# dranov/raft-tla

Measured on AMD Instinct MI355X. Metric: distinct states/sec (node) on Raft BFS, higher is better.
Workload: dtype u32

## Files before the change

raft-tla_amd/csrc/orig_backend.hip:

```cpp
#include <hip/hip_runtime.h>

#include <algorithm>
#include <chrono>
#include <cstdio>
#include <cstdlib>
#include <cstring>
#include <functional>
#include <map>
#include <sstream>
#include <type_traits>

#include "../../include/raftmc.h"
#include "backend.h"
#include "chunk_plan.h"
#include "fp_gap.h"
#include "orig_spec.h"
#include "orig_text.h"
#include "rccl_api.h"
#include "shard_transport.h"
#include "sim_rng.h"
#include "state_store.h"

namespace rmc {

enum {
  K_NEW = 0, K_GEN_IN = 1, K_ERR = 2, K_EVENT = 3, K_ERRGID = 4, K_INS = 5, K_CHUNK_NEW = 6, K_LEVEL_NEW = 7,
  K_ACT = 8, K_PROF = K_ACT + 2 * OA_NACT,
  K_PROBES = K_PROF + 6,
  K_LEAD = K_PROF + 7,
  K_NCTR = K_PROF + 8
};
enum { EV_NEXT_ERROR = 0, EV_DEADLOCK = 1, EV_INV_ERROR = 2, EV_VIOLATION = 3 };
enum { OE_CAP_STORE = 0x100, OE_TABLE_FULL = 0x200 };
constexpr int DEDUP_PER = 4;
constexpr int BS = 256;
constexpr int LDS_FP_SLOTS = 2048;
constexpr int MAT_CAP = 2048;
#ifndef RMC_RV_PATCH
#define RMC_RV_PATCH 0
#endif
#ifndef RMC_RV_WCOUNT
#define RMC_RV_WCOUNT 0
#endif
constexpr int SCAN_BS = 1024;

template <int B, int E, class F>
__device__ __forceinline__ void static_for(F&& f) {
  if constexpr (B < E) {
    f(std::integral_constant<int, B>{});
    static_for<B + 1, E>(f);
  }
}

RMC_HD u64 ev_word(u64 gid, u32 inst, u32 kind) { return (((gid << 8) | (u64)inst) << 2) | (u64)kind; }

struct GenArgs {
  const u32* states;
  u64 chunk_begin, chunk_count;
  u64 gid0;
  u64* rfp;
  unsigned short* rkey;
  u32* rcnt;
  u64 seed;
  OrigRuntime rt;
  u32 inv_oom, deadlock;
  unsigned long long* ctr;
  u32* lead;
};

template <class S>
__global__ void __launch_bounds__(BS) __attribute__((amdgpu_waves_per_eu(S::NW <= 15 ? 4 : 1))) orig_generate(GenArgs a) {
  using W = typename S::Work;
  constexpr int NW = S::NW, NWP = (S::NW + 3) & ~3;
  __shared__ unsigned int lds_cnt[OA_NACT + 1];
  for (int t = threadIdx.x; t < OA_NACT + 1; t += BS) lds_cnt[t] = 0;
  __syncthreads();
  const u64 tid = (u64)blockIdx.x * BS + threadIdx.x;
  const bool active = tid < a.chunk_count;
  const u64 gid = a.gid0 + tid;
  const int lane = __lane_id();
  const u32 wave = __builtin_amdgcn_readfirstlane(threadIdx.x >> 6);
  const u64 wreg = (u64)blockIdx.x * (BS * S::NI) + (u64)wave * (64 * S::NI);
  u64* rfp = a.rfp + wreg;
  unsigned short* rkey = a.rkey + wreg;
  u32 wcount = 0;
  W s;
  u64 al[S::AW];
  u32 err = 0, nsucc = 0, nin = 0;
  unsigned long long ev = ~0ull;
  constexpr bool INC = NW <= 16;
  u32 bw[INC ? NW : 1];
  FpBase<INC ? NW : 2> fb;
  if (active) {
    u32 w[NWP];
    const uint4* src = reinterpret_cast<const uint4*>(a.states + (a.chunk_begin + tid) * NWP);
#pragma unroll
    for (int q = 0; q < NWP / 4; ++q) { const uint4 v = src[q]; w[4 * q] = v.x; w[4 * q + 1] = v.y; w[4 * q + 2] = v.z; w[4 * q + 3] = v.w; }
    S::unpack(w, s);
    S::all_logs_next(s, al);
  } else {
    S::init(s);
#pragma unroll
    for (int q = 0; q < S::AW; ++q) al[q] = 0;
// ... 527 lines not shown
    }
  }
  u64 wm[WW];
  u32 mine = 0;
#pragma unroll
  for (int q = 0; q < WW; ++q) { wm[q] = win[threadIdx.x * WW + q]; mine += (u32)__popcll(wm[q]); }
  u32 total = 0;
  const u32 off = block_excl_scan(mine, wave_tot, &total);
  if (threadIdx.x == 0) base_sh = total ? atomicAdd(&a.ctr[K_CHUNK_NEW], (unsigned long long)total) : 0ull;
  __syncthreads();
  u64 o = base_sh + off;
  const u64 pg = a.gid0 + (u64)blockIdx.x * BS + threadIdx.x;
#pragma unroll
  for (int q = 0; q < WW; ++q) {
    u64 m = wm[q];
    while (m) {
      const int k = q * 64 + __ffsll((unsigned long long)m) - 1;
      m &= m - 1;
      a.newpos[o++] = (pg << 8) | (u64)k;
    }
  }
  if (err) atomicOr(&a.ctr[K_ERR], (unsigned long long)err);
}

struct MatPlainArgs {
  u32* states;
  u64* meta;
  const u64* newrec;
  u64 base;
  u64 dst_base, cap;
  OrigRuntime rt;
  unsigned long long* ctr;
  u32 store;
};

template <class S>
__global__ void __launch_bounds__(BS) orig_materialize_plain(MatPlainArgs a) {
  using W = typename S::Work;
  constexpr int NW = S::NW, NWP = (S::NW + 3) & ~3;
  __shared__ unsigned int lds_cnt[OA_NACT];
  for (int t = threadIdx.x; t < OA_NACT; t += BS) lds_cnt[t] = 0;
  __syncthreads();
  const u64 n_new = a.ctr[K_CHUNK_NEW];
  const u64 base = a.dst_base + a.ctr[K_LEVEL_NEW];
  u32 err = 0;
  unsigned long long ev = ~0ull;
  for (u64 i = (u64)blockIdx.x * BS + threadIdx.x; i < n_new; i += (u64)gridDim.x * BS) {
    const u64 rec = a.newrec[i], pgid = rec >> 8;
    const int k = (int)(rec & 0xff);
    u32 w[NWP];
    const uint4* src = reinterpret_cast<const uint4*>(a.states + (pgid - a.base) * NWP);
#pragma unroll
    for (int q = 0; q < NWP / 4; ++q) { const uint4 v = src[q]; w[4 * q] = v.x; w[4 * q + 1] = v.y; w[4 * q + 2] = v.z; w[4 * q + 3] = v.w; }
    W s, t;
    u64 al[S::AW];
    S::unpack(w, s);
    S::all_logs_next(s, al);
    u32 e2 = 0;
    const int act = S::apply(s, k, t, e2);
#pragma unroll
    for (int q = 0; q < S::AW; ++q) t.allLogs[q] = al[q];
    u32 pw[NW];
    S::pack(t, pw);
    const u64 dst = base + i;
    if (act >= 0 && (!a.store || dst < a.cap)) {
      if (a.store) {
        uint4* o = reinterpret_cast<uint4*>(a.states + dst * NWP);
#pragma unroll
        for (int q = 0; q < NWP / 4; ++q)
          o[q] = make_uint4(pw[4 * q], 4 * q + 1 < NW ? pw[4 * q + 1] : 0u, 4 * q + 2 < NW ? pw[4 * q + 2] : 0u, 4 * q + 3 < NW ? pw[4 * q + 3] : 0u);
        a.meta[dst] = (pgid << 24) | ((u64)act << 16) | (u64)k;
      }
      atomicAdd(&lds_cnt[act], 1u);
      if (S::violated(t, a.rt.invariants & S::inv_frame(act))) { const u64 e = ev_word(pgid, (u32)k, EV_VIOLATION); ev = e < ev ? e : ev; }
    } else {
      err |= dst >= a.cap ? (u32)OE_CAP_STORE : (u32)OE_TABLE_FULL;
    }
  }
  if (err) atomicOr(&a.ctr[K_ERR], (unsigned long long)err);
  if (ev != ~0ull) atomicMin(&a.ctr[K_EVENT], ev);
  __syncthreads();
  for (int t = threadIdx.x; t < OA_NACT; t += BS)
    if (lds_cnt[t]) atomicAdd(&a.ctr[K_ACT + OA_NACT + t], (unsigned long long)lds_cnt[t]);
}

struct MarkArgs {
  const u64* newpos;
  const u64* table;
  u64 gid0, chunk_count;
  u64* winmask;
  u32 ww;
  unsigned long long* ctr;
};

__global__ void __launch_bounds__(BS) orig_mark(MarkArgs a) {
  const u64 n = a.ctr[K_INS];
  for (u64 i = (u64)blockIdx.x * BS + threadIdx.x; i < n; i += (u64)gridDim.x * BS) {
    const u64 key = ~a.table[2 * a.newpos[i] + 1];
    const u64 p = (key >> 8) - a.gid0;
    const u32 k = (u32)(key & 255);
    if (p >= a.chunk_count) { atomicOr(&a.ctr[K_ERR], (unsigned long long)OE_TABLE_FULL); continue; }
    atomicOr((unsigned long long*)&a.winmask[p * a.ww + (k >> 6)], 1ull << (k & 63));
  }
}

template <int WW>
__global__ void __launch_bounds__(BS) orig_count(const u64* winmask, u64 chunk_count, u32* wcnt) {
  __shared__ u32 wave_tot[BS / 64];
  const u64 p = (u64)blockIdx.x * BS + threadIdx.x;
  u32 mine = 0;
#pragma unroll
  for (int q = 0; q < WW; ++q) mine += p < chunk_count ? (u32)__popcll(winmask[p * WW + q]) : 0u;
  u32 total = 0;
  (void)block_excl_scan(mine, wave_tot, &total);
  if (threadIdx.x == 0) wcnt[blockIdx.x] = total;
}

__global__ void __launch_bounds__(SCAN_BS) orig_scan(const u32* wcnt, u64* woff, u32 nblk, unsigned long long* ctr) {
  __shared__ unsigned long long part[SCAN_BS];
  const u32 per = (nblk + SCAN_BS - 1) / SCAN_BS, b0 = threadIdx.x * per;
  unsigned long long s = 0;
  for (u32 j = 0; j < per; ++j) if (b0 + j < nblk) s += wcnt[b0 + j];
  part[threadIdx.x] = s;
  __syncthreads();
  for (int d = 1; d < SCAN_BS; d <<= 1) {
    const unsigned long long x = threadIdx.x >= (unsigned)d ? part[threadIdx.x - d] : 0ull;
    __syncthreads();
    part[threadIdx.x] += x;
    __syncthreads();
  }
  unsigned long long run = part[threadIdx.x] - s;
  for (u32 j = 0; j < per; ++j) if (b0 + j < nblk) { woff[b0 + j] = run; run += wcnt[b0 + j]; }
  if (threadIdx.x == SCAN_BS - 1) ctr[K_CHUNK_NEW] = part[SCAN_BS - 1];
}

struct MatArgs {
  u32* states;
  u64* meta;
  u64 chunk_begin, chunk_count, gid0;
  u64* winmask;
  const u64* woff;
  u32 ww;
  u64 dst_base, cap;
  OrigRuntime rt;
  unsigned long long* ctr;
};

template <class S>
__global__ void __launch_bounds__(BS) orig_materialize(MatArgs a) {
  using W = typename S::Work;
  constexpr int NW = S::NW, NWP = (S::NW + 3) & ~3, WW = (S::NI + 63) / 64;
  __shared__ unsigned int lds_cnt[OA_NACT];
  __shared__ unsigned short items[MAT_CAP];
  __shared__ u32 wave_tot[BS / 64];
  for (int t = threadIdx.x; t < OA_NACT; t += BS) lds_cnt[t] = 0;
  const u64 p = (u64)blockIdx.x * BS + threadIdx.x;
  u64 wm[WW];
  u32 mine = 0;
#pragma unroll
  for (int q = 0; q < WW; ++q) {
    wm[q] = p < a.chunk_count ? a.winmask[p * WW + q] : 0ull;
    mine += (u32)__popcll(wm[q]);
  }
  if (p < a.chunk_count && mine) {
#pragma unroll
    for (int q = 0; q < WW; ++q) a.winmask[p * WW + q] = 0ull;
// ... 673 lines not shown
    if (u32 bad = S::violated(s0, m_.rt.invariants)) {
      r.verdict = MC_VERDICT_INVARIANT_VIOLATION; r.violated = first_violated(bad);
      r.trace.push_back({"<Initial predicate>", state_text(s0, true)});
      r.seconds_total = std::chrono::duration<double>(std::chrono::steady_clock::now() - t0).count();
      return 0;
    }
    struct Dev { unsigned long long* ctr = nullptr; hipEvent_t e0 = nullptr, e1 = nullptr; DevOwner<HipDevApi> own; } d;
    HIPCHK(d.own.device(&d.ctr, SK_NCTR * 8));
    HIPCHK(d.own.event(&d.e0));
    HIPCHK(d.own.event(&d.e1));
    u64 h[SK_NCTR], event = ~0ull, maxlen = 1;
    for (u64 w0 = 0; w0 < num && event == ~0ull; w0 += batch) {
      const u64 n = std::min<u64>(batch, num - w0);
      std::memset(h, 0, sizeof h);
      h[SK_EVENT] = ~0ull;
      HIPCHK(hipMemcpy(d.ctr, h, sizeof h, hipMemcpyHostToDevice));
      SimArgs a;
      a.walk0 = w0; a.nwalks = n; a.seed = o.seed; a.depth = depth; a.rt = m_.rt;
      a.inv_oom = o.inv_out_of_model ? 1u : 0u; a.deadlock = o.check_deadlock ? 1u : 0u; a.ctr = d.ctr;
      HIPCHK(hipEventRecord(d.e0, nullptr));
      hipLaunchKernelGGL((orig_simulate<S>), dim3((unsigned)((n + BS - 1) / BS)), dim3(BS), 0, nullptr, a);
      HIPCHK(hipGetLastError());
      HIPCHK(hipEventRecord(d.e1, nullptr));
      HIPCHK(hipMemcpy(h, d.ctr, sizeof h, hipMemcpyDeviceToHost));
      float ms = 0;
      HIPCHK(hipEventElapsedTime(&ms, d.e0, d.e1));
      r.kernels[0].ms += ms; r.kernels[0].launches += 1; r.n_launches += 1;
      r.seconds_kernels += ms * 1e-3;
      r.sim_walks_run += (int64_t)n;
      r.sim_steps += (int64_t)h[SK_STEPS];
      for (int k = 0; k < OA_NACT; ++k) { r.act_generated[k] += (int64_t)h[SK_ACT + k]; r.generated += (int64_t)h[SK_ACT + k]; }
      maxlen = std::max<u64>(maxlen, h[SK_MAXLEN]);
      if (progress_)
        std::fprintf(stderr, "simulation: walks %llu..%llu, %llu steps, %.3f ms\n", (unsigned long long)w0,
                     (unsigned long long)(w0 + n - 1), (unsigned long long)h[SK_STEPS], ms);
      if (h[SK_ERR]) {
        r.verdict = MC_VERDICT_CAPACITY_OVERFLOW;
        r.error = (h[SK_ERR] & OE_CAP_ELECTIONS) ? "elections set exceeds the compiled capacity" : "message count outside the packed range";
        r.depth = (int64_t)maxlen;
        r.seconds_total = std::chrono::duration<double>(std::chrono::steady_clock::now() - t0).count();
        return 0;
      }
      event = h[SK_EVENT];
    }
    r.depth = (int64_t)maxlen;
    if (event != ~0ull) {
      const u64 walk = sim_event_walk(event);
      SimWalk<S> w;
      sim_replay<S>(m_.rt, o.inv_out_of_model, o.check_deadlock, o.seed, walk, depth, w);
      if (w.event != event) {
        err = "simulation: the host replay of walk " + std::to_string(walk) + " does not reproduce the device's event";
        return MC_E_STATE;
      }
      r.sim_event_walk = (int64_t)walk;
      const u32 kind = sim_event_kind(event);
      if (kind == EV_VIOLATION) {
        r.verdict = MC_VERDICT_INVARIANT_VIOLATION;
        r.violated = first_violated(S::violated(w.states.back(), m_.rt.invariants));
      } else if (kind == EV_DEADLOCK) {
        r.verdict = MC_VERDICT_DEADLOCK;
      } else {
        r.verdict = MC_VERDICT_EVAL_ERROR;
        r.error = "TLC evaluation error while computing the successors of the last state of walk " + std::to_string(walk) +
                  ": log[i][prevLogIndex] applied outside its domain (raft_original.tla:207-210)";
      }
      for (size_t k = 0; k < w.states.size(); ++k)
        r.trace.push_back({k == 0 ? std::string("<Initial predicate>") : std::string(kOrigActNames[w.acts[k - 1]]), state_text(w.states[k], true)});
    } else {
      r.verdict = MC_VERDICT_OK;
    }
    r.seconds_total = std::chrono::duration<double>(std::chrono::steady_clock::now() - t0).count();
    return 0;
  }

  struct Search {
    std::chrono::steady_clock::time_point t0;
    bool fifo = false;
    bool count_probes = false;
    bool count_last = false;
    u64* tbl = nullptr;
    u64 tmask = 0, full_mask = 0, st_slots = 0;
    u64 level_begin = 0, level_count = 1;
    ChunkPlan plan{0, 0, 0};
    bool last = false, ovl = false;
    int nch = 0;
    u64 nnew = 0;
    double level_ms = 0;
    u64 level_end() const { return level_begin + level_count; }
  };

  int run(const RunOpts& o, RunResult& r, std::string& err) override {
    if (o.sim_walks > 0) return simulate(o, r, err);
    unstored_ = 0;
    if (int rc = ensure_alloc(o, 0, err)) return rc;
    Search s;
    s.t0 = std::chrono::steady_clock::now();
    s.fifo = o.workers == 1;
    last_fifo_ = s.fifo;
    s.count_probes = std::getenv("RAFTMC_COUNT_PROBES") != nullptr;
    if (int rc = begin_search(o, s, err)) return rc;
    r = new_result(bfs_seed(o), {"orig_generate", "orig_merge_probe", "orig_mark_scan", "orig_materialize"});
    store_.reset();
    bool ended = false;
    if (int rc = init_level0(o, s, r, ended, err)) return rc;
    if (ended) return 0;
    s.count_last = o.count_final_level && !s.fifo && o.max_depth > 0 && o.checkpoint_path.empty();
    unstored_ = 0;
    const u64 sub_env = env_u64("RAFTMC_OVERLAP_STATES", ~0ull);
    s.plan = ChunkPlan(chunk_states_, s.fifo ? 0 : sub_env == ~0ull ? ChunkPlan::default_sub(chunk_states_) : sub_env,
                       env_u64("RAFTMC_OVERLAP_MIN_LEVEL", sub_env == ~0ull ? OVERLAP_MIN_LEVEL : 0), BS);
    const u64 S_B = NWP * 4;
    while (s.level_count > 0) {
      if (o.max_depth && r.depth >= o.max_depth) { r.left_on_queue = (int64_t)s.level_count; r.verdict = MC_VERDICT_DEPTH_LIMIT; break; }
      s.last = s.count_last && r.depth + 1 >= o.max_depth;
      if (int rc = maybe_spill(s, r, err)) return rc;
      if (!ctr_clean_) {
        hipLaunchKernelGGL(orig_reset_ctr, dim3(1), dim3(64), 0, stream_, (unsigned long long*)d_ctr_);
        HIPCHK(hipGetLastError());
      }
      ctr_clean_ = false;
      if (int rc = maybe_switch_to_full_table(s, r, err)) return rc;
      if (int rc = queue_level(o, s, r, err)) return rc;
      if (int rc = read_level(s, r, err)) return rc;
      u64* const c = h_ctr_;
      const u64 level_end = s.level_end(), nnew = s.nnew;
      if (!s.last && level_end + nnew - store_.base() > store_.cap()) c[K_ERR] |= OE_CAP_STORE;
      const bool event = c[K_EVENT] != ~0ull && (c[K_ERR] & ~(u64)OE_CAP_STORE) == 0;
      if (event && !s.fifo) return research_fifo(o, c[K_EVENT], r, err);
      if (event) {
        const u64 stored = std::min<u64>(nnew, store_.cap() - std::min<u64>(store_.cap(), level_end - store_.base()));
        bool decided = false;
        if (int rc = handle_event(c[K_EVENT], s.level_begin, s.level_count, nnew, stored, r, decided, err)) return rc;
        if (decided) { store_.set_total(level_end + stored); break; }
      }
      if (c[K_ERR]) {
        r.verdict = MC_VERDICT_CAPACITY_OVERFLOW;
        r.error = capacity_error(c, level_end, nnew, r.depth);
        store_.set_total(level_end);
        r.distinct = (int64_t)level_end;
        break;
      }
      int64_t gen = 0;
      for (int k = 0; k < OA_NACT; ++k) { r.act_generated[k] += (int64_t)c[K_ACT + k]; r.act_distinct[k] += (int64_t)c[K_ACT + OA_NACT + k]; gen += (int64_t)c[K_ACT + k]; }
      r.generated += gen;
      r.generated_in_model += (int64_t)c[K_GEN_IN];
      r.seen_set_probes += (int64_t)c[K_PROBES];
      r.algo_bytes += (double)s.level_count * S_B + (double)c[K_GEN_IN] * 8 + (double)nnew * (16 + S_B);
      if (s.last) unstored_ = nnew;
      else store_.set_total(store_.total() + nnew);
      r.distinct = (int64_t)(store_.total() + unstored_);
      r.levels.back().generated = gen;
      r.levels.back().kernel_ms = s.level_ms;
      if (nnew > 0) { r.levels.push_back({(int64_t)nnew, 0, 0.0}); r.depth += 1; }
      s.level_begin += s.level_count;
      s.level_count = nnew;
      if (o.checkpoint_every > 0 && !o.checkpoint_path.empty() && r.depth % o.checkpoint_every == 0 && s.level_count > 0)
        if (int rc = save_checkpoint(o.checkpoint_path, r, s.level_begin, s.level_count, err)) return rc;
    }
    if (prof_ && prof_acc_[3])
      std::fprintf(stderr, "orig_probe per workgroup (us): %.2f  (%llu workgroups)\n",
                   prof_acc_[1] / 100.0 / prof_acc_[3], (unsigned long long)prof_acc_[3]);
    if (prof_) std::fprintf(stderr, "max concurrent dedup workgroups %llu\n", (unsigned long long)prof_acc_[4]);
    for (auto& x : prof_acc_) x = 0;
    finish(r, s.t0);
    return 0;
  }

  int begin_search(const RunOpts& o, Search& s, std::string& err) {
    s.full_mask = s.fifo ? table_mask_ : 2 * (table_mask_ + 1) - 1;
    HIPCHK(hipStreamSynchronize(clear_stream_));
    if (o.recover_path.empty()) {
      if (s.full_mask + 1 >= STARTER_FACTOR * STARTER_SLOTS) s.st_slots = STARTER_SLOTS;
      if (const char* sv = std::getenv("RAFTMC_STARTER_SLOTS")) {
        char* end = nullptr;
        const unsigned long long v = std::strtoull(sv, &end, 0);
        if (end != sv && *end == 0 && (v & (v - 1)) == 0 && (v == 0 || (v >= 64 && v <= (1ull << 32)))) s.st_slots = v;
      }
    }
    s.tbl = d_table_; s.tmask = s.full_mask;
    if (s.st_slots) {
      if (int rc = ensure_starter(s.st_slots, err)) return rc;
      HIPCHK(hipMemsetAsync(d_starter_, 0, s.st_slots * (s.fifo ? 16 : 8), stream_));
      HIPCHK(hipEventRecord(ctr_ev_, stream_));
      HIPCHK(hipStreamWaitEvent(clear_stream_, ctr_ev_, 0));
      HIPCHK(hipMemsetAsync(d_table_, 0, (table_mask_ + 1) * 16, clear_stream_));
      HIPCHK(hipEventRecord(clear_ev_, clear_stream_));
      s.tbl = d_starter_; s.tmask = s.st_slots - 1;
    } else {
      HIPCHK(hipMemsetAsync(d_table_, 0, (table_mask_ + 1) * 16, stream_));
      HIPCHK(hipStreamSynchronize(stream_));
    }
    run_table_ = s.tbl; run_mask_ = s.tmask;
    ctr_clean_ = false;
    return 0;
  }

  int init_level0(const RunOpts& o, Search& s, RunResult& r, bool& ended, std::string& err) {
    if (!o.recover_path.empty()) return load_checkpoint(o.recover_path, s.fifo, r, s.level_begin, s.level_count, err);
    W s0; S::init(s0);
    u32 w0[S::NW]; S::pack(s0, w0);
    InitWords<NWP> wp = {}; for (int q = 0; q < S::NW; ++q) wp.w[q] = w0[q];
    const u64 fp0 = fp64(w0, r.seed);
    static_assert(NWP <= 64, "orig_init_state: one lane per state word");
    if (s.fifo) hipLaunchKernelGGL((orig_init_state<NWP, 2>), dim3(1), dim3(64), 0, stream_, wp, store_.states(), store_.meta(), s.tbl, s.tmask, fp0);
    else hipLaunchKernelGGL((orig_init_state<NWP, 1>), dim3(1), dim3(64), 0, stream_, wp, store_.states(), store_.meta(), s.tbl, s.tmask, fp0);
    HIPCHK(hipGetLastError());
    r.generated = 1; r.distinct = 1; store_.set_total(1);
    r.levels.push_back({1, 1, 0.0});
    r.depth = 1;
    const u32 bad = S::violated(s0, m_.rt.invariants);
    ended = !S::in_model(s0, m_.rt) || bad;
    if (ended) HIPCHK(hipStreamSynchronize(stream_));
    if (!S::in_model(s0, m_.rt)) { err = "the initial state violates a state constraint"; r.verdict = MC_VERDICT_OK; r.distinct = 0; return 0; }
    if (bad) {
      r.verdict = MC_VERDICT_INVARIANT_VIOLATION; r.violated = first_violated(bad);
      r.trace.push_back({"<Initial predicate>", state_text(s0, true)});
      finish(r, s.t0);
    }
    return 0;
  }

  int maybe_spill(const Search& s, const RunResult& r, std::string& err) {
    if (s.level_begin <= store_.base() || s.last) return 0;
    const double prev = r.levels.size() >= 2 ? (double)r.levels[r.levels.size() - 2].states : 1.0;
    const double pred = (double)s.level_count * std::max(1.0, (double)s.level_count / std::max(prev, 1.0)) * 1.5;
    if ((double)(store_.total() - store_.base()) + pred <= (double)store_.cap()) return 0;
    if (progress_) std::fprintf(stderr, "spilling %llu completed states to host memory\n", (unsigned long long)(s.level_begin - store_.base()));
    return store_.spill(s.level_begin, s.level_count, stream_, progress_, err);
  }

  int maybe_switch_to_full_table(Search& s, const RunResult& r, std::string& err) {
    if (s.tbl != d_starter_ || s.level_end() + s.level_count * (u64)S::NI <= s.st_slots / 2) return 0;
    HIPCHK(hipStreamWaitEvent(stream_, clear_ev_, 0));
    unsigned long long* const moved = progress_ ? (unsigned long long*)d_stop_ : nullptr;
    if (moved) HIPCHK(hipMemsetAsync(d_stop_, 0, 8, stream_));
    const unsigned mblk = (unsigned)std::min<u64>(2048, (s.st_slots + BS - 1) / BS);
    if (s.fifo) hipLaunchKernelGGL((orig_migrate<2>), dim3(mblk), dim3(BS), 0, stream_, (const u64*)d_starter_, s.st_slots, d_table_, s.full_mask, (unsigned long long*)d_ctr_, moved);
    else hipLaunchKernelGGL((orig_migrate<1>), dim3(mblk), dim3(BS), 0, stream_, (const u64*)d_starter_, s.st_slots, d_table_, s.full_mask, (unsigned long long*)d_ctr_, moved);
    HIPCHK(hipGetLastError());
    if (moved) {
      u64 n = 0;
      HIPCHK(hipMemcpyAsync(&n, d_stop_, 8, hipMemcpyDeviceToHost, stream_));
      HIPCHK(hipStreamSynchronize(stream_));
      std::fprintf(stderr, "seen-set switch after level %lld: %llu entries moved from the %llu-slot starter to the full table\n",
                   (long long)r.depth, (unsigned long long)n, (unsigned long long)s.st_slots);
    }
    s.tbl = d_table_; s.tmask = s.full_mask;
    run_table_ = s.tbl; run_mask_ = s.tmask;
    return 0;
  }

  int queue_level(const RunOpts& o, Search& s, RunResult& r, std::string& err) {
    s.ovl = s.plan.plan(s.level_count, chunks_);
    const int nchunks = (int)chunks_.size();
    hipStream_t const gst = s.ovl ? clear_stream_ : stream_;
    for (s.nch = 0; s.nch < nchunks; ++s.nch) {
      const int q = s.nch;
      const u64 cb = s.level_begin + chunks_[q].first, cnt = chunks_[q].count;
      const u64 rec0 = chunks_[q].buffer ? s.plan.half_cap : 0;
      const unsigned nblk = (unsigned)((cnt + BS - 1) / BS);
      hipEvent_t e[8];
      for (int j = 0; j < 8; ++j) e[j] = pool_ev(8 * q + j);
      if (!e[7]) { err = "hipEventCreate failed"; return MC_E_NO_DEVICE; }
      const GenArgs g = gen_args(cb - store_.base(), cnt, cb, r.seed, o, rec0);
      if (s.ovl && q == 0) {
        HIPCHK(hipEventRecord(gen_ev_, stream_));
        HIPCHK(hipStreamWaitEvent(gst, gen_ev_, 0));
      }
      if (s.ovl && q >= 2) HIPCHK(hipStreamWaitEvent(gst, pool_ev(8 * (q - 2) + 3), 0));
      HIPCHK(hipEventRecord(e[0], gst));
      launch_generate(g, nblk, gst);
      HIPCHK(hipGetLastError());
      HIPCHK(hipEventRecord(e[1], gst));
      if (s.ovl) {
        if (q + 1 < nchunks) HIPCHK(hipMemsetAsync(d_ctr_ + K_LEAD, 0, 8, gst));
        HIPCHK(hipStreamWaitEvent(stream_, e[1], 0));
        HIPCHK(hipEventRecord(e[2], stream_));
      }
      const DedupArgs d = dedup_args(g, cb, s.tbl, s.tmask);
      if (s.fifo) { if (int rc = queue_merge_probe(s, d, nblk, err)) return rc; }
      else launch_dedup_plain(d, nblk, s.ovl && q + 1 < nchunks ? OVERLAP_DEDUP_PAD_LDS : 0u, s.count_probes);
      HIPCHK(hipGetLastError());
      HIPCHK(hipEventRecord(e[3], stream_));
      if (s.fifo) { if (int rc = queue_winners_materialize(s, cb, cnt, nblk, e[5], err)) return rc; }
      else launch_materialize_plain(mat_plain_args(store_.base(), s.level_end() - store_.base(), !s.last), cnt);
      HIPCHK(hipGetLastError());
      HIPCHK(hipEventRecord(e[7], stream_));
      if (q + 1 < nchunks) {
        hipLaunchKernelGGL(orig_advance, dim3(1), dim3(64), 0, stream_, (unsigned long long*)d_ctr_, s.ovl ? 0 : 1);
        HIPCHK(hipGetLastError());
      }
      for (size_t k = 0; k < r.kernels.size(); ++k) if (s.fifo || k != 2) r.kernels[k].launches += 1;
      r.kernels[0].algo_bytes += (double)cnt * NWP * 4;
    }
    return 0;
  }

  int queue_merge_probe(const Search& s, const DedupArgs& d, unsigned nblk, std::string& err) {
    hipLaunchKernelGGL(orig_merge, dim3(nblk), dim3(BS), 0, stream_, d);
    HIPCHK(hipGetLastError());
    if (s.count_probes) hipLaunchKernelGGL((orig_probe<true>), dim3(nblk), dim3(BS), 0, stream_, d);
    else hipLaunchKernelGGL((orig_probe<false>), dim3(nblk), dim3(BS), 0, stream_, d);
    return 0;
  }

  int queue_winners_materialize(const Search& s, u64 cb, u64 cnt, unsigned nblk, hipEvent_t e5, std::string& err) {
    MarkArgs mk;
    mk.newpos = d_newrec_; mk.table = s.tbl; mk.gid0 = cb; mk.chunk_count = cnt; mk.winmask = d_winmask_;
    mk.ww = WW; mk.ctr = (unsigned long long*)d_ctr_;
    hipLaunchKernelGGL(orig_mark, dim3((unsigned)std::min<u64>(2048, (cnt * 2 + BS - 1) / BS)), dim3(BS), 0, stream_, mk);
    HIPCHK(hipGetLastError());
    hipLaunchKernelGGL((orig_count<WW>), dim3(nblk), dim3(BS), 0, stream_, (const u64*)d_winmask_, cnt, d_wcnt_);
    HIPCHK(hipGetLastError());
    hipLaunchKernelGGL(orig_scan, dim3(1), dim3(SCAN_BS), 0, stream_, (const u32*)d_wcnt_, d_woff_, (u32)nblk, (unsigned long long*)d_ctr_);
    HIPCHK(hipGetLastError());
    HIPCHK(hipEventRecord(e5, stream_));
    MatArgs m;
    m.states = store_.states(); m.meta = store_.meta(); m.chunk_begin = cb - store_.base(); m.chunk_count = cnt; m.gid0 = cb;
    m.winmask = d_winmask_; m.woff = d_woff_; m.ww = WW; m.dst_base = s.level_end() - store_.base(); m.cap = store_.cap();
    m.rt = m_.rt; m.ctr = (unsigned long long*)d_ctr_;
    hipLaunchKernelGGL((orig_materialize<S>), dim3(nblk), dim3(BS), 0, stream_, m);
    return 0;
  }

  int read_level(Search& s, RunResult& r, std::string& err) {
    u64* const c = h_ctr_;
    HIPCHK(hipMemcpyAsync(c, d_ctr_, K_NCTR * 8, hipMemcpyDeviceToHost, stream_));
    HIPCHK(hipEventRecord(ctr_ev_, stream_));
    hipLaunchKernelGGL(orig_reset_ctr, dim3(1), dim3(64), 0, stream_, (unsigned long long*)d_ctr_);
    HIPCHK(hipGetLastError());
    ctr_clean_ = true;
    HIPCHK(hipEventSynchronize(ctr_ev_));
    const bool fifo = s.fifo, last = s.last;
    const u64 level_end = s.level_end(), S_B = NWP * 4;
    double level_ms = 0;
    for (int q = 0; q < s.nch; ++q) {
      const std::pair<int, int> pr[4] = {{0, 1}, {s.ovl ? 2 : 1, 3}, {3, fifo ? 5 : 3}, {fifo ? 5 : 3, 7}};
      for (int k = 0; k < 4; ++k) {
        float ms = 0;
        if (pr[k].first != pr[k].second) (void)hipEventElapsedTime(&ms, pool_ev(8 * q + pr[k].first), pool_ev(8 * q + pr[k].second));
        r.kernels[k].ms += ms; level_ms += ms;
      }
    }
    const u64 nnew = c[K_LEVEL_NEW] + c[K_CHUNK_NEW];
    const u64 next_write = level_end + nnew;
    if (progress_)
      std::fprintf(stderr, "Progress(%lld) at %.3f s: %lld states generated, %llu distinct states found, %llu states left on queue "
                           "(level kernels %.1f ms, %d chunk(s), store %llu/%llu, %llu on the host%s)\n",
                   (long long)r.depth + 1,
                   std::chrono::duration<double>(std::chrono::steady_clock::now() - s.t0).count(),
                   (long long)(r.generated + (int64_t)[&] { u64 g = 0; for (int k = 0; k < OA_NACT; ++k) g += c[K_ACT + k]; return g; }()),
                   (unsigned long long)(level_end + nnew), (unsigned long long)nnew, level_ms, s.nch,
                   (unsigned long long)((last ? level_end : next_write) - store_.base()), (unsigned long long)store_.cap(), (unsigned long long)store_.base(),
                   last ? "; the last level counted, not stored" : "");
    if (progress_ && (c[K_EVENT] != ~0ull || c[K_ERR]))
      std::fprintf(stderr, "level %lld: event word 0x%llx, error flags 0x%llx\n", (long long)r.depth + 1,
                   (unsigned long long)c[K_EVENT], (unsigned long long)c[K_ERR]);
    if (prof_) {
      for (int q = 0; q < 4; ++q) prof_acc_[q] += c[K_PROF + q];
      prof_acc_[4] = std::max<u64>(prof_acc_[4], c[K_PROF + 5]);
    }
    const u64 G_in = c[K_GEN_IN];
    r.kernels[0].algo_bytes += (double)G_in * 10;
    r.kernels[1].algo_bytes += (double)G_in * (10 + 8) + (double)nnew * (16 + 8);
    r.kernels[2].algo_bytes += (double)nnew * (8 + 16 + 8);
    r.kernels[3].algo_bytes += (double)s.level_count * WW * 8 + (double)nnew * (S_B + S_B + 8);
    r.seconds_kernels += level_ms / 1000.0;
    r.n_launches += 1;
    s.nnew = nnew; s.level_ms = level_ms;
    return 0;
  }

  int research_fifo(const RunOpts& o, u64 evw, RunResult& r, std::string& err) {
    RunOpts o1 = o;
    o1.workers = 1;
    o1.recover_path.clear();
    o1.checkpoint_path.clear();
    const int64_t ev_depth = r.depth + 1;
    const int rc = run(o1, r, err);
    if (rc == 0 && r.verdict == MC_VERDICT_CAPACITY_OVERFLOW) {
      static const char* const kind[4] = {"an evaluation error", "a deadlock", "an invariant evaluation error", "an invariant violation"};
      r.error = std::string("the -workers N search found ") + kind[evw & 3] + " at depth " + std::to_string(ev_depth) +
                "; TLC's single-worker re-search of it (for TLC's counterexample and stop point) ran out of capacity: " + r.error;
    }
    return rc;
  }

  std::string capacity_error(const u64* c, u64 level_end, u64 nnew, int64_t depth) const {
    const u64 e = c[K_ERR];
    std::ostringstream os;
    os << "error flags 0x" << std::hex << e << std::dec << " while expanding state " << (c[K_ERRGID] ? (int64_t)(c[K_ERRGID] - 1) : -1) << ":";
    if (e & OE_CAP_ELECTIONS) os << " elections set exceeds the compiled capacity;";
    if (e & OE_CAP_COUNT) os << " message count / bag capacity exceeded;";
    if (e & OE_CAP_STORE)
      os << " state store full (raise state_store_bytes): " << store_.cap() << " state slots, " << store_.base()
         << " states on the host, level ends at " << level_end << ", " << nnew << " new;";
    if (e & OE_TABLE_FULL) os << " fingerprint table full (raise fp_table_bytes);";
    os << " the summary counts the " << level_end << " states of the " << depth << " completed levels;";
    return os.str();
  }

  int handle_event(u64 ev, u64 level_begin, u64 level_count, u64 nnew, u64 stored, RunResult& r, bool& decided,
                   std::string& err) {
    const int kind = (int)(ev & 3);
    const u64 key = ev >> 2, pg = key >> 8;
    const u32 k = (u32)(key & 255);
    const u64 level_end = level_begin + level_count;
    auto key_at = [&](u64 i, u64& kk) -> int {
      u64 mt = 0;
      HIPCHK(hipMemcpy(&mt, store_.meta() + (level_end - store_.base()) + i, 8, hipMemcpyDeviceToHost));
      kk = ((mt >> 24) << 8) | (mt & 0xff);
      return 0;
    };
    u64 lo = 0, hi = stored;
    while (lo < hi) {
      const u64 mid = (lo + hi) / 2;
      u64 kk = 0;
      if (int rc = key_at(mid, kk)) return rc;
      const bool before = kk < key || (kk == key && kind >= EV_INV_ERROR);
      if (before) lo = mid + 1; else hi = mid;
    }
    const u64 before = lo;
    decided = before < stored || stored == nnew;
    const auto te0 = std::chrono::steady_clock::now();
    auto since = [&]() { return std::chrono::duration<double>(std::chrono::steady_clock::now() - te0).count(); };
    if (progress_)
      std::fprintf(stderr, "event kind %d at parent %llu instance %u: %llu new states before it (%s)\n", kind,
                   (unsigned long long)pg, k, (unsigned long long)before, decided ? "decided" : "beyond the stored states");
    if (!decided) return 0;
    (void)nnew;
    HIPCHK(hipMemsetAsync(d_stop_, 0, (1 + OA_NACT) * 8, stream_));
    const u64 npar = pg - level_begin + 1;
    hipLaunchKernelGGL((orig_stop_generated<S>), dim3((unsigned)((npar + BS - 1) / BS)), dim3(BS), 0, stream_,
                       (const u32*)store_.states(), level_begin - store_.base(), npar, level_begin, pg, k, (u32)kind, (unsigned long long*)d_stop_);
    HIPCHK(hipGetLastError());
    u64 gs[1 + OA_NACT];
    HIPCHK(hipMemcpyAsync(gs, d_stop_, sizeof gs, hipMemcpyDeviceToHost, stream_));
    HIPCHK(hipStreamSynchronize(stream_));
    HIPCHK(hipMemsetAsync(d_stop_, 0, (1 + OA_NACT) * 8, stream_));
    if (before)
      hipLaunchKernelGGL(orig_stop_distinct, dim3((unsigned)((before + BS - 1) / BS)), dim3(BS), 0, stream_,
                         (const u64*)(store_.meta() + (level_end - store_.base())), before, (unsigned long long*)d_stop_);
    HIPCHK(hipGetLastError());
    u64 ds[1 + OA_NACT];
    HIPCHK(hipMemcpyAsync(ds, d_stop_, sizeof ds, hipMemcpyDeviceToHost, stream_));
    HIPCHK(hipStreamSynchronize(stream_));
    if (progress_) std::fprintf(stderr, "stop-point counters over %llu parents: %.3f s\n", (unsigned long long)npar, since());
    r.generated += (int64_t)gs[0];
    for (int a = 0; a < OA_NACT; ++a) { r.act_generated[a] += (int64_t)gs[1 + a]; r.act_distinct[a] += (int64_t)ds[a]; }
// ... 554 lines not shown
```

Measured before the change: 2.432 billion.

## Add fused single-kernel path for small BFS levels

Adds an orig_small_level kernel that handles a whole BFS level in one launch: it generates successors, probes the seen-set table and stores new states directly. Levels at or below a threshold (default 32768 states, non-FIFO, not last, not instrumented) take this path instead of the multi-kernel generate/merge/mark/materialize pipeline. The aim is to cut per-level launch and synchronisation overhead on the many small early levels. The trade-offs are per-item atomics for slot allocation, possibly different output ordering of new states, and a second code path to maintain.

```diff
diff --git a/raft-tla_amd/csrc/orig_backend.hip b/raft-tla_amd/csrc/orig_backend.hip
--- a/raft-tla_amd/csrc/orig_backend.hip
+++ b/raft-tla_amd/csrc/orig_backend.hip
@@ -19,6 +19,7 @@
 #include "rccl_api.h"
 #include "shard_transport.h"
 #include "sim_rng.h"
+#include "small_level.h"
 #include "state_store.h"
 
 namespace rmc {
@@ -712,6 +713,115 @@
   __syncthreads();
   for (int t = threadIdx.x; t < OA_NACT; t += BS)
     if (lds_cnt[t]) atomicAdd(&a.ctr[K_ACT + OA_NACT + t], (unsigned long long)lds_cnt[t]);
+}
+
+struct SmallArgs {
+  u32* states;
+  u64* meta;
+  u64 level_begin, level_count;
+  u64 gid0;
+  u64 dst_base, cap;
+  u64* table;
+  u64 table_mask;
+  u64 seed;
+  OrigRuntime rt;
+  u32 inv_oom, deadlock;
+  unsigned long long* ctr;
+};
+
+template <class S, int NWAVES>
+__global__ void __launch_bounds__(64 * NWAVES) orig_small_level(SmallArgs a) {
+  using W = typename S::Work;
+  constexpr int NW = S::NW, NWP = (S::NW + 3) & ~3;
+  __shared__ unsigned int lds_cnt[2 * OA_NACT + 1];
+  __shared__ unsigned int lds_succ[SMALL_PARENTS];
+  for (int t = threadIdx.x; t < 2 * OA_NACT + 1; t += 64 * NWAVES) lds_cnt[t] = 0;
+  if (threadIdx.x < SMALL_PARENTS) lds_succ[threadIdx.x] = 0;
+  __syncthreads();
+  const int lane = __lane_id();
+  const int wave = (int)__builtin_amdgcn_readfirstlane(threadIdx.x >> 6);
+  const u64 p = small_level_parent(blockIdx.x, lane);
+  const bool active = p < a.level_count;
+  const u64 gid = a.gid0 + p;
+  W s;
+  u64 al[S::AW];
+  if (active) {
+    u32 w[NWP];
+    const uint4* src = reinterpret_cast<const uint4*>(a.states + (a.level_begin + p) * NWP);
+#pragma unroll
+    for (int q = 0; q < NWP / 4; ++q) { const uint4 v = src[q]; w[4 * q] = v.x; w[4 * q + 1] = v.y; w[4 * q + 2] = v.z; w[4 * q + 3] = v.w; }
+    S::unpack(w, s);
+    S::all_logs_next(s, al);
+  } else {
+    S::init(s);
+#pragma unroll
+    for (int q = 0; q < S::AW; ++q) al[q] = 0;
+  }
+  u32 err = 0, nsucc = 0, nin = 0;
+  unsigned long long ev = ~0ull;
+#pragma unroll 1
+  for (int trip = 0; trip < small_level_trips(S::NI, NWAVES); ++trip) {
+    const int k = small_level_instance(wave, trip, NWAVES);
+    if (k >= S::NI) break;
+    W t;
+    u32 pw[NW];
+    u64 fp = 0;
+    u32 what = 0;
+    const int act = active ? small_level_item<S>(s, al, k, a.rt, a.inv_oom != 0, a.seed, t, pw, fp, err, what) : -1;
+    if (act >= 0) {
+      ++nsucc;
+      atomicAdd(&lds_cnt[act], 1u);
+    }
+    if (what & SI_OOM_BAD) { const u64 e = ev_word(gid, (u32)k, EV_VIOLATION); ev = e < ev ? e : ev; }
+    bool inserted = false;
+    if (what & SI_IN_MODEL) {
+      ++nin;
+      const u64 f[1] = {fp}, nk[1] = {0ull};
+      u64 pos[1];
+      inserted = probe_batch<1, false, 1>(a.table, a.table_mask, f, nk, pos, err) != 0u;
+    }
+    const u64 im = __ballot(inserted);
+    if (im) {
+      const int first = __ffsll((unsigned long long)im) - 1;
+      u32 blo = 0, bhi = 0;
+      if (lane == first) {
+        const unsigned long long b = atomicAdd(&a.ctr[K_CHUNK_NEW], (unsigned long long)__popcll(im));
+        blo = (u32)b; bhi = (u32)(b >> 32);
+      }
+      blo = __shfl(blo, first); bhi = __shfl(bhi, first);
+      if (inserted) {
+        const u64 slot = (((u64)bhi << 32) | blo) + __builtin_amdgcn_mbcnt_hi((u32)(im >> 32), __builtin_amdgcn_mbcnt_lo((u32)im, 0u));
+        const u64 dst = a.dst_base + slot;
+        if (dst < a.cap) {
+          uint4* o = reinterpret_cast<uint4*>(a.states + dst * NWP);
+#pragma unroll
+          for (int q = 0; q < NWP / 4; ++q)
+            o[q] = make_uint4(pw[4 * q], 4 * q + 1 < NW ? pw[4 * q + 1] : 0u, 4 * q + 2 < NW ? pw[4 * q + 2] : 0u, 4 * q + 3 < NW ? pw[4 * q + 3] : 0u);
+          a.meta[dst] = (gid << 24) | ((u64)act << 16) | (u64)k;
+          atomicAdd(&lds_cnt[OA_NACT + act], 1u);
+          if (S::violated(t, a.rt.invariants & S::inv_frame(act))) { const u64 e = ev_word(gid, (u32)k, EV_VIOLATION); ev = e < ev ? e : ev; }
+        } else {
+          err |= (u32)OE_CAP_STORE;
+        }
+      }
+    }
+  }
+  if (nsucc) atomicAdd(&lds_succ[lane], nsucc);
+  if (nin) atomicAdd(&lds_cnt[2 * OA_NACT], nin);
+  __syncthreads();
+  if (active) {
+    if (err & OE_EVAL_LOG_INDEX) { const u64 e = ev_word(gid, 0, EV_NEXT_ERROR); ev = e < ev ? e : ev; }
+    if (wave == 0 && a.deadlock && lds_succ[lane] == 0) { const u64 e = ev_word(gid, 0, EV_DEADLOCK); ev = e < ev ? e : ev; }
+  }
+  const u32 cap_err = err & ~(u32)OE_EVAL_LOG_INDEX;
+  if (cap_err) {
+    atomicOr(&a.ctr[K_ERR], (unsigned long long)cap_err);
+    if (cap_err & (OE_CAP_ELECTIONS | OE_CAP_COUNT)) atomicCAS(&a.ctr[K_ERRGID], 0ull, (unsigned long long)(gid + 1));
+  }
+  if (ev != ~0ull) atomicMin(&a.ctr[K_EVENT], ev);
+  for (int t = threadIdx.x; t < 2 * OA_NACT; t += 64 * NWAVES)
+    if (lds_cnt[t]) atomicAdd(&a.ctr[K_ACT + t], (unsigned long long)lds_cnt[t]);
+  if (threadIdx.x == 0 && lds_cnt[2 * OA_NACT]) atomicAdd(&a.ctr[K_GEN_IN], (unsigned long long)lds_cnt[2 * OA_NACT]);
 }
 
 struct MarkArgs {
@@ -1551,7 +1661,8 @@
     u64 tmask = 0, full_mask = 0, st_slots = 0;
     u64 level_begin = 0, level_count = 1;
     ChunkPlan plan{0, 0, 0};
-    bool last = false, ovl = false;
+    bool last = false, ovl = false, small = false;
+    u64 small_states = 0;
     int nch = 0;
     u64 nnew = 0;
     double level_ms = 0;
@@ -1568,7 +1679,9 @@
     last_fifo_ = s.fifo;
     s.count_probes = std::getenv("RAFTMC_COUNT_PROBES") != nullptr;
     if (int rc = begin_search(o, s, err)) return rc;
-    r = new_result(bfs_seed(o), {"orig_generate", "orig_merge_probe", "orig_mark_scan", "orig_materialize"});
+    s.small_states = s.fifo ? 0 : small_level_threshold(s.full_mask + 1, STARTER_FACTOR * STARTER_SLOTS, env_u64("RAFTMC_SMALL_LEVEL_STATES", ~0ull));
+    if (s.small_states) r = new_result(bfs_seed(o), {"orig_generate", "orig_merge_probe", "orig_mark_scan", "orig_materialize", "orig_small_level"});
+    else r = new_result(bfs_seed(o), {"orig_generate", "orig_merge_probe", "orig_mark_scan", "orig_materialize"});
     store_.reset();
     bool ended = false;
     if (int rc = init_level0(o, s, r, ended, err)) return rc;
@@ -1720,6 +1833,8 @@
   }
 
   int queue_level(const RunOpts& o, Search& s, RunResult& r, std::string& err) {
+    s.small = small_level_use(s.level_count, s.small_states, s.fifo, s.last, s.count_probes || prof_);
+    if (s.small) return queue_small_level(o, s, r, err);
     s.ovl = s.plan.plan(s.level_count, chunks_);
     const int nchunks = (int)chunks_.size();
     hipStream_t const gst = s.ovl ? clear_stream_ : stream_;
@@ -1759,9 +1874,28 @@
         hipLaunchKernelGGL(orig_advance, dim3(1), dim3(64), 0, stream_, (unsigned long long*)d_ctr_, s.ovl ? 0 : 1);
         HIPCHK(hipGetLastError());
       }
-      for (size_t k = 0; k < r.kernels.size(); ++k) if (s.fifo || k != 2) r.kernels[k].launches += 1;
+      for (size_t k = 0; k < 4; ++k) if (s.fifo || k != 2) r.kernels[k].launches += 1;
       r.kernels[0].algo_bytes += (double)cnt * NWP * 4;
     }
+    return 0;
+  }
+
+  int queue_small_level(const RunOpts& o, Search& s, RunResult& r, std::string& err) {
+    s.ovl = false; s.nch = 0;
+    hipEvent_t const e0 = pool_ev(0), e1 = pool_ev(1);
+    if (!e0 || !e1) { err = "hipEventCreate failed"; return MC_E_NO_DEVICE; }
+    SmallArgs a;
+    a.states = store_.states(); a.meta = store_.meta();
+    a.level_begin = s.level_begin - store_.base(); a.level_count = s.level_count; a.gid0 = s.level_begin;
+    a.dst_base = s.level_end() - store_.base(); a.cap = store_.cap();
+    a.table = s.tbl; a.table_mask = s.tmask; a.seed = r.seed; a.rt = m_.rt;
+    a.inv_oom = o.inv_out_of_model ? 1u : 0u; a.deadlock = o.check_deadlock ? 1u : 0u;
+    a.ctr = (unsigned long long*)d_ctr_;
+    HIPCHK(hipEventRecord(e0, stream_));
+    hipLaunchKernelGGL((orig_small_level<S, SMALL_WAVES>), dim3((unsigned)small_level_grid(s.level_count)), dim3(64 * SMALL_WAVES), 0, stream_, a);
+    HIPCHK(hipGetLastError());
+    HIPCHK(hipEventRecord(e1, stream_));
+    r.kernels[4].launches += 1;
     return 0;
   }
 
@@ -1811,6 +1945,11 @@
         r.kernels[k].ms += ms; level_ms += ms;
       }
     }
+    if (s.small) {
+      float ms = 0;
+      (void)hipEventElapsedTime(&ms, pool_ev(0), pool_ev(1));
+      r.kernels[4].ms += ms; level_ms += ms;
+    }
     const u64 nnew = c[K_LEVEL_NEW] + c[K_CHUNK_NEW];
     const u64 next_write = level_end + nnew;
     if (progress_)
@@ -1830,10 +1969,14 @@
       prof_acc_[4] = std::max<u64>(prof_acc_[4], c[K_PROF + 5]);
     }
     const u64 G_in = c[K_GEN_IN];
-    r.kernels[0].algo_bytes += (double)G_in * 10;
-    r.kernels[1].algo_bytes += (double)G_in * (10 + 8) + (double)nnew * (16 + 8);
-    r.kernels[2].algo_bytes += (double)nnew * (8 + 16 + 8);
-    r.kernels[3].algo_bytes += (double)s.level_count * WW * 8 + (double)nnew * (S_B + S_B + 8);
+    if (s.small) {
+      r.kernels[4].algo_bytes += (double)s.level_count * S_B + (double)G_in * 8 + (double)nnew * (16 + S_B);
+    } else {
+      r.kernels[0].algo_bytes += (double)G_in * 10;
+      r.kernels[1].algo_bytes += (double)G_in * (10 + 8) + (double)nnew * (16 + 8);
+      r.kernels[2].algo_bytes += (double)nnew * (8 + 16 + 8);
+      r.kernels[3].algo_bytes += (double)s.level_count * WW * 8 + (double)nnew * (S_B + S_B + 8);
+    }
     r.seconds_kernels += level_ms / 1000.0;
     r.n_launches += 1;
     s.nnew = nnew; s.level_ms = level_ms;
diff --git a/raft-tla_amd/csrc/small_level.h b/raft-tla_amd/csrc/small_level.h
--- /dev/null
+++ b/raft-tla_amd/csrc/small_level.h
@@ -0,0 +1,52 @@
+#pragma once
+#include <cstdint>
+
+#include "orig_spec.h"
+
+namespace rmc {
+
+constexpr int SMALL_PARENTS = 64;
+#ifndef RMC_SMALL_WAVES
+#define RMC_SMALL_WAVES 8
+#endif
+constexpr int SMALL_WAVES = RMC_SMALL_WAVES;
+constexpr uint64_t SMALL_LEVEL_STATES = 32768;
+constexpr uint64_t SMALL_LEVEL_MAX = 1ull << 32;
+
+inline uint64_t small_level_threshold(uint64_t table_slots, uint64_t starter_min_slots, uint64_t env) {
+  const uint64_t v = env != ~0ull ? env : table_slots >= starter_min_slots ? SMALL_LEVEL_STATES : 0;
+  return v < SMALL_LEVEL_MAX ? v : SMALL_LEVEL_MAX;
+}
+
+inline bool small_level_use(uint64_t level_count, uint64_t small_states, bool fifo, bool last, bool instrumented) {
+  return !fifo && !last && !instrumented && level_count > 0 && level_count <= small_states;
+}
+
+inline uint64_t small_level_grid(uint64_t level_count) { return (level_count + SMALL_PARENTS - 1) / SMALL_PARENTS; }
+
+RMC_HD uint64_t small_level_parent(uint64_t wg, int lane) { return wg * SMALL_PARENTS + (uint64_t)lane; }
+RMC_HD int small_level_instance(int wave, int trip, int waves) { return wave + trip * waves; }
+RMC_HD int small_level_trips(int ni, int waves) { return (ni + waves - 1) / waves; }
+
+enum { SI_COUNTED = 1, SI_IN_MODEL = 2, SI_OOM_BAD = 4 };
+template <class S>
+RMC_HD int small_level_item(const typename S::Work& s, const u64 (&al)[S::AW], int k, const OrigRuntime& rt, bool inv_oom, u64 seed,
+                            typename S::Work& t, u32 (&pw)[S::NW], u64& fp, u32& err, u32& what) {
+  what = 0;
+  const int qa = S::quick_out_of_model(s, k, rt);
+  if (qa >= 0) { what = SI_COUNTED; return qa; }
+  const int act = S::apply(s, k, t, err);
+  if (act < 0) return -1;
+#pragma unroll
+  for (int q = 0; q < S::AW; ++q) t.allLogs[q] = al[q];
+  if (S::in_model(t, rt)) {
+    S::pack(t, pw);
+    fp = fp64(pw, seed);
+    what = SI_IN_MODEL;
+  } else if (inv_oom && S::violated(t, rt.invariants & S::inv_frame(act))) {
+    what = SI_OOM_BAD;
+  }
+  return act;
+}
+
+}
```

Result: no change. 2.443 billion (median of 4 runs) (+0.4%).
